# Plonky3/Plonky3-recursion

Hardware: AMD Instinct MI355X
Metric: prove_next_layer ms + Poseidon2 perms/s, KoalaBear 2^20-row circuit, 1/8 GPU (lower is better)
Workload: dtype u32 Montgomery (31-bit prime field, degree-4 extension); Poseidon2 hashing as exact integers in f64; 1 GPU; prove_next_layer (verifier-circuit run on the device + prove_all_tables) of the synthetic koala-bear 2^20-row recursion layer: tables const/public/alu/poseidon2/recompose, FRI blowup 4, arity<=4, 54 queries, 15-bit PoW; circuit inputs + NextLayerPrepCache resident in HBM; field=koala-bear, log_height=20, independent_proofs=1, proof_bytes=612900, parallelism=1 independent proofs, one per GPU, no data-path collective

## Files before the change

plonky3_recursion_amd/csrc/field.h:

```cpp
#pragma once
#include <type_traits>
#include <stdint.h>

#if defined(__HIPCC__)
#include <hip/hip_runtime.h>
#define P3R_HD __host__ __device__ __forceinline__
#else
#define P3R_HD inline
#endif

namespace p3r {

#if defined(__HIPCC__)
template <class T>
using gptr = T __attribute__((address_space(1)))*;
template <class T>
__device__ __forceinline__ gptr<T> as_global(T* p) {
  return (gptr<T>)p;
}

template <class Job>
__device__ __forceinline__ int find_job(const Job* __restrict__ jobs, int n_jobs) {
  int lo = 0, hi = n_jobs - 1;
  while (lo < hi) {
// ... 32 lines not shown
};
struct BabyBearParams {
  static constexpr uint32_t P = 0x78000001u;
  static constexpr uint32_t GEN = 31;
  static constexpr int TWO_ADICITY = 27;
  static constexpr uint32_t EXT_W = 11;
  static constexpr int SBOX_DEGREE = 7;
  static constexpr int SBOX_REGISTERS = 1;
  static constexpr int PARTIAL_ROUNDS = 13;
  static constexpr int PARTIAL_ROUNDS_W32 = 30;
  static constexpr int FIELD_ID = 1;
};

template <class PP>
struct Fp {
  using Params = PP;
  static constexpr uint32_t P = PP::P;
  static constexpr uint32_t MU = inv_mod_2_32(PP::P);
  static constexpr uint32_t R1 = (uint32_t)((1ull << 32) % PP::P);
  static constexpr uint32_t R2 = (uint32_t)((uint64_t)R1 * R1 % PP::P);

  uint32_t v;

  static P3R_HD uint32_t mulhi(uint32_t a, uint32_t b) {
#if defined(__HIP_DEVICE_COMPILE__)
    return __umulhi(a, b);
#else
    return (uint32_t)(((uint64_t)a * b) >> 32);
#endif
  }
  static constexpr uint32_t NEG_MU = 0u - MU;
  static P3R_HD uint32_t reduce64(uint64_t x) {
#if defined(__HIP_DEVICE_COMPILE__)
    const uint32_t q = (uint32_t)x * NEG_MU;
    const uint32_t r = (uint32_t)(((uint64_t)q * P + x) >> 32);
    const uint32_t r2 = r - P;
    return r < r2 ? r : r2;
#else
    const uint32_t lo = (uint32_t)x, hi = (uint32_t)(x >> 32);
    uint32_t t = lo * MU;
    uint32_t u = mulhi(t, P);
    uint32_t r = hi - u;
    return hi < u ? r + P : r;
#endif
  }
  static P3R_HD uint32_t reduce(uint32_t lo, uint32_t hi) { return reduce64(((uint64_t)hi << 32) | lo); }
  static P3R_HD uint32_t reduce64_lazy(uint64_t x) {
#if defined(__HIP_DEVICE_COMPILE__)
    const uint32_t q = (uint32_t)x * NEG_MU;
    return (uint32_t)(((uint64_t)q * P + x) >> 32);
#else
    return reduce64(x);
#endif
  }
  P3R_HD Fp sqr_times(Fp x) const {
    const uint32_t sq = reduce64_lazy((uint64_t)v * v);
    return raw(reduce64((uint64_t)sq * x.v));
  }
  P3R_HD Fp cube() const {
    const uint32_t sq = reduce64_lazy((uint64_t)v * v);
    return raw(reduce64((uint64_t)sq * v));
  }
  static P3R_HD Fp raw(uint32_t m) { Fp r; r.v = m; return r; }
  static P3R_HD Fp zero() { return raw(0); }
  static P3R_HD Fp one() { return raw(R1); }
  static P3R_HD Fp from_canonical(uint32_t x) {
    return raw(reduce64((uint64_t)x * R2));
  }
  static P3R_HD Fp from_u64(uint64_t x) { return from_canonical((uint32_t)(x % P)); }
  P3R_HD uint32_t to_canonical() const { return reduce(v, 0); }

  friend P3R_HD Fp operator+(Fp a, Fp b) {
    uint32_t s = a.v + b.v;
    return raw(s >= P ? s - P : s);
  }
  friend P3R_HD Fp operator-(Fp a, Fp b) {
    uint32_t d = a.v - b.v;
    return raw(a.v < b.v ? d + P : d);
  }
  friend P3R_HD Fp operator*(Fp a, Fp b) { return raw(reduce64((uint64_t)a.v * b.v)); }
  static P3R_HD Fp dot2(Fp a1, Fp b1, Fp a2, Fp b2) {
    return raw(reduce64((uint64_t)a1.v * b1.v + (uint64_t)a2.v * b2.v));
  }
  P3R_HD Fp operator-() const { return raw(v ? P - v : 0); }
  P3R_HD Fp& operator+=(Fp o) { *this = *this + o; return *this; }
  P3R_HD Fp& operator-=(Fp o) { *this = *this - o; return *this; }
  P3R_HD Fp& operator*=(Fp o) { *this = *this * o; return *this; }
  P3R_HD bool operator==(Fp o) const { return v == o.v; }
  P3R_HD bool operator!=(Fp o) const { return v != o.v; }
  P3R_HD Fp dbl() const { return *this + *this; }
  P3R_HD Fp sqr() const { return *this * *this; }
  P3R_HD Fp halve() const {
    uint32_t t = (v & 1) ? v + P : v;
    return raw(t >> 1);
  }
  P3R_HD Fp pow(uint64_t e) const {
    Fp r = one(), b = *this;
    while (e) {
      if (e & 1) r *= b;
      b = b.sqr();
      e >>= 1;
    }
    return r;
  }
  P3R_HD Fp inv() const { return pow((uint64_t)P - 2); }

  static P3R_HD Fp generator() { return from_canonical(PP::GEN); }
  static P3R_HD Fp two_adic_generator(int bits) {
    Fp g = from_canonical(PP::GEN).pow(((uint64_t)P - 1) >> PP::TWO_ADICITY);
    for (int i = PP::TWO_ADICITY; i > bits; --i) g = g.sqr();
    return g;
  }
};

template <class PP>
struct Fp4 {
  using F = Fp<PP>;
  F c[4];

  static P3R_HD Fp4 zero() { Fp4 r; r.c[0] = r.c[1] = r.c[2] = r.c[3] = F::zero(); return r; }
  static P3R_HD Fp4 one() { Fp4 r = zero(); r.c[0] = F::one(); return r; }
  static P3R_HD Fp4 from_base(F b) { Fp4 r = zero(); r.c[0] = b; return r; }
  static P3R_HD F w() { return F::from_canonical(PP::EXT_W); }

  friend P3R_HD Fp4 operator+(Fp4 a, Fp4 b) {
    Fp4 r;
    for (int i = 0; i < 4; ++i) r.c[i] = a.c[i] + b.c[i];
    return r;
  }
  friend P3R_HD Fp4 operator-(Fp4 a, Fp4 b) {
    Fp4 r;
    for (int i = 0; i < 4; ++i) r.c[i] = a.c[i] - b.c[i];
    return r;
  }
  P3R_HD Fp4 operator-() const {
    Fp4 r;
    for (int i = 0; i < 4; ++i) r.c[i] = -c[i];
    return r;
  }
  friend P3R_HD Fp4 operator*(Fp4 a, Fp4 b) {
    const F W = w();
    const F wa1 = W * a.c[1], wa2 = W * a.c[2], wa3 = W * a.c[3];
    Fp4 r;
    r.c[0] = F::dot2(a.c[0], b.c[0], wa1, b.c[3]) + F::dot2(wa2, b.c[2], wa3, b.c[1]);
    r.c[1] = F::dot2(a.c[0], b.c[1], a.c[1], b.c[0]) + F::dot2(wa2, b.c[3], wa3, b.c[2]);
    r.c[2] = F::dot2(a.c[0], b.c[2], a.c[1], b.c[1]) + F::dot2(a.c[2], b.c[0], wa3, b.c[3]);
    r.c[3] = F::dot2(a.c[0], b.c[3], a.c[1], b.c[2]) + F::dot2(a.c[2], b.c[1], a.c[3], b.c[0]);
    return r;
  }
  friend P3R_HD Fp4 operator*(Fp4 a, F b) {
    Fp4 r;
    for (int i = 0; i < 4; ++i) r.c[i] = a.c[i] * b;
    return r;
  }
  static P3R_HD Fp4 dot2_base(const Fp4& a1, F b1, const Fp4& a2, F b2) {
    Fp4 r;
    for (int i = 0; i < 4; ++i) r.c[i] = F::dot2(a1.c[i], b1, a2.c[i], b2);
    return r;
  }
  P3R_HD Fp4& operator+=(Fp4 o) { *this = *this + o; return *this; }
  P3R_HD Fp4& operator-=(Fp4 o) { *this = *this - o; return *this; }
  P3R_HD Fp4& operator*=(Fp4 o) { *this = *this * o; return *this; }
  P3R_HD bool operator==(const Fp4& o) const {
    return c[0] == o.c[0] && c[1] == o.c[1] && c[2] == o.c[2] && c[3] == o.c[3];
  }
  P3R_HD bool is_zero() const { return (c[0].v | c[1].v | c[2].v | c[3].v) == 0; }
  P3R_HD Fp4 sqr() const { return *this * *this; }
  P3R_HD Fp4 dbl() const { Fp4 r; for (int i = 0; i < 4; ++i) r.c[i] = c[i].dbl(); return r; }
  P3R_HD Fp4 halve() const { Fp4 r; for (int i = 0; i < 4; ++i) r.c[i] = c[i].halve(); return r; }
  P3R_HD Fp4 pow(uint64_t e) const {
    Fp4 r = one(), b = *this;
    while (e) {
      if (e & 1) r *= b;
      b = b.sqr();
      e >>= 1;
    }
    return r;
  }
  struct Norm { F n0, n1, d; };
  P3R_HD Norm norm() const {
    const F W = w();
    F A0 = c[0] * c[0] + W * (c[2] * c[2]);
    F A1 = (c[0] * c[2]).dbl();
    F B0 = c[1] * c[1] + W * (c[3] * c[3]);
    F B1 = (c[1] * c[3]).dbl();
    Norm r;
    r.n0 = A0 - W * B1;
    r.n1 = A1 - B0;
    r.d = r.n0 * r.n0 - W * (r.n1 * r.n1);
    return r;
  }
  P3R_HD Fp4 inv() const {
    const Norm nm = norm();
    return inv_given(nm, nm.d.inv());
  }
  P3R_HD Fp4 inv_given(const Norm& nm, F d) const {
    const F W = w();
    F i0 = nm.n0 * d;
    F i1 = -(nm.n1 * d);
    Fp4 r;
    r.c[0] = c[0] * i0 + W * (c[2] * i1);
    r.c[2] = c[0] * i1 + c[2] * i0;
    r.c[1] = -(c[1] * i0 + W * (c[3] * i1));
    r.c[3] = -(c[1] * i1 + c[3] * i0);
    return r;
  }
};

template <class PP>
inline constexpr bool kHasQuintic = PP::P == 0x7f000001u;
template <class PP>
struct Fp1 {
  using F = Fp<PP>;
  F c[1];
  static P3R_HD Fp1 zero() { Fp1 r; r.c[0] = F::zero(); return r; }
  friend P3R_HD Fp1 operator+(Fp1 a, Fp1 b) { Fp1 r; r.c[0] = a.c[0] + b.c[0]; return r; }
  friend P3R_HD Fp1 operator-(Fp1 a, Fp1 b) { Fp1 r; r.c[0] = a.c[0] - b.c[0]; return r; }
  friend P3R_HD Fp1 operator*(Fp1 a, Fp1 b) { Fp1 r; r.c[0] = a.c[0] * b.c[0]; return r; }
  static P3R_HD Fp1 one() { Fp1 r; r.c[0] = F::one(); return r; }
  static P3R_HD Fp1 from_base(F b) { Fp1 r; r.c[0] = b; return r; }
  P3R_HD bool operator==(const Fp1& o) const { return c[0] == o.c[0]; }
  P3R_HD Fp1 inv() const { Fp1 r; r.c[0] = c[0].inv(); return r; }
};
template <class PP, class Fn>
inline void dispatch_ext_degree(int d, Fn&& fn) {
  if (d == 1) fn(std::integral_constant<int, 1>{});
  else if (d == 5) { if constexpr (kHasQuintic<PP>) fn(std::integral_constant<int, 5>{}); }
  else fn(std::integral_constant<int, 4>{});
}
template <class PP, class Fn>
inline void dispatch_air_degree(int d, Fn&& fn) {
  if (d == 2) fn(std::integral_constant<int, 2>{});
  else if (d == 6) fn(std::integral_constant<int, 6>{});
  else if (d == 8) fn(std::integral_constant<int, 8>{});
  else dispatch_ext_degree<PP>(d, fn);
}
inline bool ext_degree_is_binomial_generic(uint32_t d) { return d == 2 || d == 6 || d == 8; }

namespace quintic {
struct Q5 { uint64_t c[5]; };
constexpr Q5 q5_mul(Q5 a, Q5 b, uint64_t p) {
  uint64_t t[9] = {0, 0, 0, 0, 0, 0, 0, 0, 0};
  for (int i = 0; i < 5; ++i)
    for (int j = 0; j < 5; ++j) t[i + j] = (t[i + j] + a.c[i] * b.c[j] % p) % p;
  for (int k = 8; k >= 5; --k) {
    t[k - 5] = (t[k - 5] + t[k]) % p;
    t[k - 3] = (t[k - 3] + p - t[k]) % p;
  }
  return Q5{{t[0], t[1], t[2], t[3], t[4]}};
}
constexpr Q5 q5_pow(Q5 b, uint64_t e, uint64_t p) {
  Q5 r{{1, 0, 0, 0, 0}};
  while (e) {
    if (e & 1) r = q5_mul(r, b, p);
    b = q5_mul(b, b, p);
    e >>= 1;
  }
  return r;
}
constexpr uint32_t frob_entry(uint32_t p, int k, int i, int j) {
  Q5 x{{0, 1, 0, 0, 0}};
  for (int s = 0; s < k; ++s) x = q5_pow(x, p, p);
  const Q5 xi = q5_pow(x, (uint64_t)i, p);
  return (uint32_t)((xi.c[j] << 32) % p);
}
}
template <class PP, int K, int I, int J>
inline constexpr uint32_t kFrob5 = quintic::frob_entry(PP::P, K, I, J);

template <class PP>
struct Fp5 {
  using F = Fp<PP>;
  F c[5];
  static P3R_HD Fp5 zero() { Fp5 r; for (int i = 0; i < 5; ++i) r.c[i] = F::zero(); return r; }
  friend P3R_HD Fp5 operator+(Fp5 a, Fp5 b) { Fp5 r; for (int i = 0; i < 5; ++i) r.c[i] = a.c[i] + b.c[i]; return r; }
  friend P3R_HD Fp5 operator-(Fp5 a, Fp5 b) { Fp5 r; for (int i = 0; i < 5; ++i) r.c[i] = a.c[i] - b.c[i]; return r; }
  friend P3R_HD Fp5 operator*(Fp5 a, Fp5 b) {
    const F c5 = F::dot2(a.c[1], b.c[4], a.c[2], b.c[3]) + F::dot2(a.c[3], b.c[2], a.c[4], b.c[1]);
    const F c6 = F::dot2(a.c[2], b.c[4], a.c[3], b.c[3]) + a.c[4] * b.c[2];
    const F c7 = F::dot2(a.c[3], b.c[4], a.c[4], b.c[3]);
    const F c8 = a.c[4] * b.c[4];
    const F c58 = c5 - c8;
    Fp5 r;
    r.c[0] = a.c[0] * b.c[0] + c58;
    r.c[1] = F::dot2(a.c[0], b.c[1], a.c[1], b.c[0]) + c6;
    r.c[2] = F::dot2(a.c[0], b.c[2], a.c[1], b.c[1]) + a.c[2] * b.c[0] - c58 + c7;
    r.c[3] = F::dot2(a.c[0], b.c[3], a.c[1], b.c[2]) + F::dot2(a.c[2], b.c[1], a.c[3], b.c[0]) - c6 + c8;
    r.c[4] = F::dot2(a.c[0], b.c[4], a.c[1], b.c[3]) + F::dot2(a.c[2], b.c[2], a.c[3], b.c[1]) + a.c[4] * b.c[0] - c7;
    return r;
  }
  friend P3R_HD Fp5 operator*(Fp5 a, F b) { Fp5 r; for (int i = 0; i < 5; ++i) r.c[i] = a.c[i] * b; return r; }
  P3R_HD Fp5 operator-() const { Fp5 r; for (int i = 0; i < 5; ++i) r.c[i] = -c[i]; return r; }
  P3R_HD Fp5& operator+=(Fp5 o) { *this = *this + o; return *this; }
  P3R_HD Fp5& operator-=(Fp5 o) { *this = *this - o; return *this; }
  P3R_HD Fp5& operator*=(Fp5 o) { *this = *this * o; return *this; }
  P3R_HD bool is_zero() const { return (c[0].v | c[1].v | c[2].v | c[3].v | c[4].v) == 0; }
  P3R_HD Fp5 sqr() const { return *this * *this; }
  P3R_HD Fp5 dbl() const { Fp5 r; for (int i = 0; i < 5; ++i) r.c[i] = c[i].dbl(); return r; }
  P3R_HD Fp5 halve() const { Fp5 r; for (int i = 0; i < 5; ++i) r.c[i] = c[i].halve(); return r; }
  P3R_HD Fp5 pow(uint64_t e) const {
    Fp5 r = one(), b = *this;
    while (e) {
      if (e & 1) r *= b;
      b = b.sqr();
      e >>= 1;
    }
    return r;
  }
  static P3R_HD Fp5 dot2_base(const Fp5& a1, F b1, const Fp5& a2, F b2) {
    Fp5 r;
    for (int i = 0; i < 5; ++i) r.c[i] = F::dot2(a1.c[i], b1, a2.c[i], b2);
    return r;
  }
  static P3R_HD Fp5 one() { Fp5 r = zero(); r.c[0] = F::one(); return r; }
  static P3R_HD Fp5 from_base(F b) { Fp5 r = zero(); r.c[0] = b; return r; }
  P3R_HD bool operator==(const Fp5& o) const {
    return c[0] == o.c[0] && c[1] == o.c[1] && c[2] == o.c[2] && c[3] == o.c[3] && c[4] == o.c[4];
  }
  template <int K, int J>
  P3R_HD F frobenius_coeff() const {
    const F t = F::dot2(c[1], F::raw(kFrob5<PP, K, 1, J>), c[2], F::raw(kFrob5<PP, K, 2, J>)) +
                F::dot2(c[3], F::raw(kFrob5<PP, K, 3, J>), c[4], F::raw(kFrob5<PP, K, 4, J>));
    return J == 0 ? c[0] + t : t;
  }
  template <int K>
  P3R_HD Fp5 frobenius() const {
    Fp5 r;
    r.c[0] = frobenius_coeff<K, 0>();
    r.c[1] = frobenius_coeff<K, 1>();
    r.c[2] = frobenius_coeff<K, 2>();
    r.c[3] = frobenius_coeff<K, 3>();
    r.c[4] = frobenius_coeff<K, 4>();
    return r;
  }
  static P3R_HD F mul_c0(const Fp5& a, const Fp5& b) {
    return a.c[0] * b.c[0] + F::dot2(a.c[1], b.c[4], a.c[2], b.c[3]) + F::dot2(a.c[3], b.c[2], a.c[4], b.c[1]) -
           a.c[4] * b.c[4];
  }
  P3R_HD Fp5 norm_cofactor() const {
    const Fp5 a1 = frobenius<1>();
    const Fp5 t = a1 * a1.template frobenius<1>();
    return t * t.template frobenius<2>();
  }
  P3R_HD Fp5 inv() const {
    const Fp5 co = norm_cofactor();
    return co * mul_c0(*this, co).inv();
  }
};

template <class PP, int D> struct CircuitExt;
template <class PP> struct CircuitExt<PP, 1> { using type = Fp1<PP>; };
template <class PP> struct CircuitExt<PP, 4> { using type = Fp4<PP>; };
template <class PP> struct CircuitExt<PP, 5> { using type = Fp5<PP>; };

template <class V> struct Lift;
template <class PP> struct Lift<Fp<PP>> { static P3R_HD Fp<PP> of(Fp<PP> x) { return x; } };
template <class PP> struct Lift<Fp4<PP>> { static P3R_HD Fp4<PP> of(Fp<PP> x) { return Fp4<PP>::from_base(x); } };
template <class PP> struct Lift<Fp5<PP>> { static P3R_HD Fp5<PP> of(Fp<PP> x) { return Fp5<PP>::from_base(x); } };
template <class PP, int DC> struct Chal;
template <class PP> struct Chal<PP, 4> { using type = Fp4<PP>; };
template <class PP> struct Chal<PP, 5> { using type = Fp5<PP>; };

P3R_HD uint32_t bit_reverse(uint32_t x, int bits) {
  if (bits == 0) return 0;
#if defined(__HIP_DEVICE_COMPILE__)
  return __brev(x) >> (32 - bits);
#else
  uint32_t r = 0;
  for (int i = 0; i < bits; ++i) r |= ((x >> i) & 1u) << (bits - 1 - i);
  return r;
#endif
}

}
```

plonky3_recursion_amd/csrc/field_test_ops.h:

```cpp
#pragma once
#include "field.h"

namespace p3r {

enum FieldTestOp : int {
  FT_FP_ADD = 0,
  FT_FP_SUB = 1,
  FT_FP_NEG = 2,
  FT_FP_MUL = 3,
  FT_FP_SQR = 4,
  FT_FP_DBL = 5,
  FT_FP_HALVE = 6,
  FT_FP_DOT2 = 7,
  FT_FP_SQR_TIMES = 8,
  FT_FP_CUBE = 9,
  FT_FP_REDUCE_LAZY = 10,
  FT_FP_FROM_CANONICAL = 11,
  FT_FP_TO_CANONICAL = 12,
  FT_FP_POW = 13,
  FT_FP_INV = 14,
  FT_FP_TWO_ADIC_GEN = 15,
  FT_BIT_REVERSE = 16,

  FT_FP4_ADD = 32,
  FT_FP4_SUB = 33,
  FT_FP4_NEG = 34,
  FT_FP4_MUL = 35,
  FT_FP4_MUL_BASE = 36,
  FT_FP4_DOT2_BASE = 37,
  FT_FP4_SQR = 38,
  FT_FP4_DBL = 39,
  FT_FP4_HALVE = 40,
  FT_FP4_POW = 41,
  FT_FP4_NORM = 42,
  FT_FP4_INV_GIVEN = 43,
  FT_FP4_INV = 44,

  FT_FP5_ADD = 64,
  FT_FP5_SUB = 65,
  FT_FP5_NEG = 66,
  FT_FP5_MUL = 67,
  FT_FP5_MUL_BASE = 68,
  FT_FP5_DOT2_BASE = 69,
  FT_FP5_SQR = 70,
  FT_FP5_FROBENIUS1 = 71,
  FT_FP5_FROBENIUS2 = 72,
  FT_FP5_MUL_C0 = 73,
  FT_FP5_NORM_COFACTOR = 74,
  FT_FP5_POW = 75,
  FT_FP5_INV = 76,
  FT_FP5_DBL = 77,
  FT_FP5_HALVE = 78,

  FT_FP1_MUL = 96,
  FT_FP1_INV = 97,
};

P3R_HD bool field_test_shape(int op, int* words_in, int* words_out) {
  int wi = 0, wo = 0;
  switch (op) {
    case FT_FP_ADD: case FT_FP_SUB: case FT_FP_MUL: case FT_FP_SQR_TIMES: case FT_FP_REDUCE_LAZY: case FT_BIT_REVERSE:
      wi = 2, wo = 1; break;
    case FT_FP_NEG: case FT_FP_SQR: case FT_FP_DBL: case FT_FP_HALVE: case FT_FP_CUBE: case FT_FP_FROM_CANONICAL:
    case FT_FP_TO_CANONICAL: case FT_FP_POW: case FT_FP_INV: case FT_FP_TWO_ADIC_GEN:
      wi = 1, wo = 1; break;
    case FT_FP_DOT2: wi = 4, wo = 1; break;
    case FT_FP4_ADD: case FT_FP4_SUB: case FT_FP4_MUL: wi = 8, wo = 4; break;
    case FT_FP4_NEG: case FT_FP4_SQR: case FT_FP4_DBL: case FT_FP4_HALVE: case FT_FP4_POW: case FT_FP4_INV: wi = 4, wo = 4; break;
    case FT_FP4_MUL_BASE: case FT_FP4_INV_GIVEN: wi = 5, wo = 4; break;
    case FT_FP4_DOT2_BASE: wi = 10, wo = 4; break;
    case FT_FP4_NORM: wi = 4, wo = 3; break;
    case FT_FP5_ADD: case FT_FP5_SUB: case FT_FP5_MUL: wi = 10, wo = 5; break;
    case FT_FP5_NEG: case FT_FP5_SQR: case FT_FP5_FROBENIUS1: case FT_FP5_FROBENIUS2: case FT_FP5_NORM_COFACTOR:
    case FT_FP5_POW: case FT_FP5_INV: case FT_FP5_DBL: case FT_FP5_HALVE:
      wi = 5, wo = 5; break;
    case FT_FP5_MUL_BASE: wi = 6, wo = 5; break;
    case FT_FP5_DOT2_BASE: wi = 12, wo = 5; break;
    case FT_FP5_MUL_C0: wi = 10, wo = 1; break;
    case FT_FP1_MUL: wi = 2, wo = 1; break;
    case FT_FP1_INV: wi = 1, wo = 1; break;
    default: return false;
  }
  *words_in = wi;
  *words_out = wo;
  return true;
}
P3R_HD bool field_test_is_quintic(int op) { return op >= FT_FP5_ADD && op <= FT_FP5_HALVE; }

template <class E, int D>
P3R_HD E field_test_load(const uint32_t* in) {
  E e;
  for (int i = 0; i < D; ++i) e.c[i].v = in[i];
  return e;
}
template <class E, int D>
P3R_HD void field_test_store(uint32_t* out, const E& e) {
  for (int i = 0; i < D; ++i) out[i] = e.c[i].v;
}

template <class PP>
P3R_HD bool field_test_apply(int op, const uint32_t* in, uint32_t* out, uint32_t aux) {
  using F = Fp<PP>;
  using E4 = Fp4<PP>;
  using E1 = Fp1<PP>;
  auto f = [&](int i) { return F::raw(in[i]); };
  auto e4 = [&](int i) { return field_test_load<E4, 4>(in + i); };
  auto put4 = [&](const E4& e) { field_test_store<E4, 4>(out, e); };
  switch (op) {
    case FT_FP_ADD: out[0] = (f(0) + f(1)).v; return true;
    case FT_FP_SUB: out[0] = (f(0) - f(1)).v; return true;
    case FT_FP_NEG: out[0] = (-f(0)).v; return true;
    case FT_FP_MUL: out[0] = (f(0) * f(1)).v; return true;
    case FT_FP_SQR: out[0] = f(0).sqr().v; return true;
    case FT_FP_DBL: out[0] = f(0).dbl().v; return true;
    case FT_FP_HALVE: out[0] = f(0).halve().v; return true;
    case FT_FP_DOT2: out[0] = F::dot2(f(0), f(1), f(2), f(3)).v; return true;
    case FT_FP_SQR_TIMES: out[0] = f(0).sqr_times(f(1)).v; return true;
    case FT_FP_CUBE: out[0] = f(0).cube().v; return true;
    case FT_FP_REDUCE_LAZY: out[0] = F::reduce64_lazy((uint64_t)in[0] * in[1]); return true;
    case FT_FP_FROM_CANONICAL: out[0] = F::from_canonical(in[0]).v; return true;
    case FT_FP_TO_CANONICAL: out[0] = f(0).to_canonical(); return true;
    case FT_FP_POW: out[0] = f(0).pow(aux).v; return true;
    case FT_FP_INV: out[0] = f(0).inv().v; return true;
    case FT_FP_TWO_ADIC_GEN: out[0] = F::two_adic_generator((int)in[0]).v; return true;
    case FT_BIT_REVERSE: out[0] = bit_reverse(in[0], (int)in[1]); return true;

    case FT_FP4_ADD: put4(e4(0) + e4(4)); return true;
    case FT_FP4_SUB: put4(e4(0) - e4(4)); return true;
    case FT_FP4_NEG: put4(-e4(0)); return true;
    case FT_FP4_MUL: put4(e4(0) * e4(4)); return true;
    case FT_FP4_MUL_BASE: put4(e4(0) * f(4)); return true;
    case FT_FP4_DOT2_BASE: put4(E4::dot2_base(e4(0), f(4), e4(5), f(9))); return true;
    case FT_FP4_SQR: put4(e4(0).sqr()); return true;
    case FT_FP4_DBL: put4(e4(0).dbl()); return true;
    case FT_FP4_HALVE: put4(e4(0).halve()); return true;
    case FT_FP4_POW: put4(e4(0).pow(aux)); return true;
    case FT_FP4_NORM: {
      const typename E4::Norm nm = e4(0).norm();
      out[0] = nm.n0.v, out[1] = nm.n1.v, out[2] = nm.d.v;
      return true;
    }
    case FT_FP4_INV_GIVEN: {
      const E4 a = e4(0);
      put4(a.inv_given(a.norm(), f(4)));
      return true;
    }
    case FT_FP4_INV: put4(e4(0).inv()); return true;

    case FT_FP1_MUL: field_test_store<E1, 1>(out, field_test_load<E1, 1>(in) * field_test_load<E1, 1>(in + 1)); return true;
    case FT_FP1_INV: field_test_store<E1, 1>(out, field_test_load<E1, 1>(in).inv()); return true;
    default: break;
  }
  if constexpr (kHasQuintic<PP>) {
    using E5 = Fp5<PP>;
    auto e5 = [&](int i) { return field_test_load<E5, 5>(in + i); };
    auto put5 = [&](const E5& e) { field_test_store<E5, 5>(out, e); };
    switch (op) {
      case FT_FP5_ADD: put5(e5(0) + e5(5)); return true;
      case FT_FP5_SUB: put5(e5(0) - e5(5)); return true;
      case FT_FP5_NEG: put5(-e5(0)); return true;
      case FT_FP5_MUL: put5(e5(0) * e5(5)); return true;
      case FT_FP5_MUL_BASE: put5(e5(0) * f(5)); return true;
      case FT_FP5_DOT2_BASE: put5(E5::dot2_base(e5(0), f(5), e5(6), f(11))); return true;
      case FT_FP5_SQR: put5(e5(0).sqr()); return true;
      case FT_FP5_FROBENIUS1: put5(e5(0).template frobenius<1>()); return true;
      case FT_FP5_FROBENIUS2: put5(e5(0).template frobenius<2>()); return true;
      case FT_FP5_MUL_C0: out[0] = E5::mul_c0(e5(0), e5(5)).v; return true;
      case FT_FP5_NORM_COFACTOR: put5(e5(0).norm_cofactor()); return true;
      case FT_FP5_POW: put5(e5(0).pow(aux)); return true;
      case FT_FP5_INV: put5(e5(0).inv()); return true;
      case FT_FP5_DBL: put5(e5(0).dbl()); return true;
      case FT_FP5_HALVE: put5(e5(0).halve()); return true;
      default: break;
    }
  }
  return false;
}

}
```

plonky3_recursion_amd/csrc/kernels_fri_points.hip.h:

```cpp
#pragma once
#include "kernels_fri_reduce.hip.h"

namespace p3r {

template <int DC>
struct FriPointT {
  const uint32_t* inv;
  const uint32_t* v;
  EW<DC> off;
};
struct FriPointsMat {
  const uint32_t* mat;
  int w;
  uint32_t p0, n_points;
};
template <class PP, int DC = 4>
__global__ void __launch_bounds__(kBlock)
k_fri_reduce_points(const FriReduceJob* __restrict__ jobs, int n_jobs, const FriPointsMat* __restrict__ mats,
                    const FriPointT<DC>* __restrict__ pts, const uint32_t* __restrict__ apow_tab ) {
  using F = Fp<PP>;
  using E = typename Chal<PP, DC>::type;
  const int j = find_job(jobs, n_jobs);
  const FriReduceJob job = jobs[j];
  const size_t h = job.h, r = (size_t)(blockIdx.x - job.block0) * kBlock + threadIdx.x;
  if (r >= h) return;
  auto apow = [&](int c) {
    E ap;
#pragma unroll
    for (int k = 0; k < DC; ++k) ap.c[k] = F::raw(apow_tab[DC * c + k]);
    return ap;
  };
  E acc = E::zero();
  for (uint32_t m = 0; m < job.n_mats; ++m) {
    const FriPointsMat a = mats[job.mat0 + m];
    const gptr<const uint32_t> mat = as_global(a.mat);
    const int w = a.w;
    E S = E::zero(), S2 = E::zero();
    int c = 0;
    for (; c + 3 < w; c += 4) {
      const F m0 = F::raw(mat[(size_t)c * h + r]), m1 = F::raw(mat[(size_t)(c + 1) * h + r]);
      const F m2 = F::raw(mat[(size_t)(c + 2) * h + r]), m3 = F::raw(mat[(size_t)(c + 3) * h + r]);
      S += E::dot2_base(apow(c), m0, apow(c + 1), m1);
      S2 += E::dot2_base(apow(c + 2), m2, apow(c + 3), m3);
    }
    for (; c + 1 < w; c += 2)
      S += E::dot2_base(apow(c), F::raw(mat[(size_t)c * h + r]), apow(c + 1), F::raw(mat[(size_t)(c + 1) * h + r]));
    if (c < w) S += apow(c) * F::raw(mat[(size_t)c * h + r]);
    S += S2;
    for (uint32_t p = 0; p < a.n_points; ++p) {
      const FriPointT<DC>& q = pts[a.p0 + p];
      E inv, V;
#pragma unroll
      for (int k = 0; k < DC; ++k) inv.c[k] = F::raw(as_global(q.inv)[(size_t)k * h + r]);
#pragma unroll
      for (int k = 0; k < DC; ++k) V.c[k] = F::raw(as_global(q.v)[k]);
      acc += e4_load<PP, DC>(q.off) * (V - S) * inv;
    }
  }
#pragma unroll
  for (int k = 0; k < DC; ++k) as_global(job.ro)[(size_t)k * h + r] = acc.c[k].v;
}

template <int DC, int LA>
__global__ void __launch_bounds__(kBlock) k_fri_leaf_view(const uint32_t* __restrict__ in, uint32_t* __restrict__ out, size_t rows) {
  static_assert(LA >= 1 && LA <= 4, "rows of 2, 4, 8 or 16 elements");
  constexpr int ARITY = 1 << LA;
  const size_t r = (size_t)blockIdx.x * kBlock + threadIdx.x;
  const int k = (int)blockIdx.y;
  if (r >= rows) return;
  const size_t n_in = rows << LA;
  const gptr<const uint32_t> src = as_global(in) + (size_t)k * n_in + (r << LA);
  uint32_t e[ARITY];
  if constexpr (LA == 1) {
    const fri_u32x2 v = *(gptr<const fri_u32x2>)src;
    e[0] = v.x;
    e[1] = v.y;
  } else {
#pragma unroll
    for (int q = 0; q < ARITY / 4; ++q) {
      const fri_u32x4 v = ((gptr<const fri_u32x4>)src)[q];
      e[4 * q] = v.x;
      e[4 * q + 1] = v.y;
      e[4 * q + 2] = v.z;
      e[4 * q + 3] = v.w;
    }
  }
  const gptr<uint32_t> dst = as_global(out) + (size_t)k * rows + r;
#pragma unroll
  for (int j = 0; j < ARITY; ++j) dst[(size_t)j * DC * rows] = e[j];
}

}
```

plonky3_recursion_amd/csrc/kernels_fri_reduce.hip.h:

```cpp
#pragma once
#include "kernels_stark.hip.h"

namespace p3r {

template <int DC>
struct FriInvJobT {
  uint32_t* inv;
  uint64_t h;
  int log_h;
  uint32_t w_h;
  uint32_t w_4;
  EW<DC> z;
  uint32_t block0;
};
using FriInvJob = FriInvJobT<4>;
template <class PP, int DC = 4>
__global__ void __launch_bounds__(kBlock)
k_fri_inv_points(const FriInvJobT<DC>* __restrict__ jobs, int n_jobs, uint32_t gen) {
  using F = Fp<PP>;
  using E = typename Chal<PP, DC>::type;
  const int j = find_job(jobs, n_jobs);
  const FriInvJobT<DC>& job = jobs[j];
  const size_t h = job.h, r0 = ((size_t)(blockIdx.x - job.block0) * kBlock + threadIdx.x) * 4;
  if (r0 >= h) return;
  const E z = e4_load<PP, DC>(job.z);
  E x[4], v[4];
  const F x0 = F::raw(gen) * F::raw(job.w_h).pow(bit_reverse((uint32_t)r0, job.log_h));
  const F x2 = x0 * F::raw(job.w_4);
  x[0] = z - E::from_base(x0);
  x[1] = z + E::from_base(x0);
  x[2] = z - E::from_base(x2);
  x[3] = z + E::from_base(x2);
  inv4<PP>(x, v);
  const gptr<uint32_t> inv = as_global(job.inv);
#pragma unroll
  for (int m = 0; m < 4; ++m)
    if (r0 + m < h)
#pragma unroll
      for (int k = 0; k < DC; ++k) inv[(size_t)k * h + r0 + m] = v[m].c[k].v;
}

struct FriVsumJob {
  const uint32_t* vals;
  uint32_t* out;
  int w;
};
template <class PP, int DC = 4>
__global__ void __launch_bounds__(kBlock)
k_fri_vsum(const FriVsumJob* __restrict__ jobs, const uint32_t* __restrict__ apow_tab ) {
  using F = Fp<PP>;
  using E = typename Chal<PP, DC>::type;
  __shared__ uint32_t sh[kBlock / 64][DC];
  const FriVsumJob job = jobs[blockIdx.x];
  const gptr<const uint32_t> vals = as_global(job.vals);
  E acc = E::zero();
  for (int c = threadIdx.x; c < job.w; c += kBlock) {
    E ap, v;
#pragma unroll
    for (int k = 0; k < DC; ++k) {
      ap.c[k] = F::raw(apow_tab[DC * c + k]);
      v.c[k] = F::raw(vals[DC * c + k]);
    }
    acc += ap * v;
  }
  const int lane = threadIdx.x & 63, wave = threadIdx.x >> 6;
#pragma unroll
  for (int k = 0; k < DC; ++k) {
    F x = acc.c[k];
#pragma unroll
    for (int off = 32; off > 0; off >>= 1) x += F::raw(__shfl_down(x.v, off));
    if (lane == 0) sh[wave][k] = x.v;
  }
  __syncthreads();
  if (threadIdx.x < DC) {
    F x = F::zero();
#pragma unroll
    for (int wv = 0; wv < kBlock / 64; ++wv) x += F::raw(sh[wv][threadIdx.x]);
    as_global(job.out)[threadIdx.x] = x.v;
  }
}

template <int DC>
struct FriReduceMatT {
  const uint32_t* mat;
  int w, n_points;
  const uint32_t* inv[2];
  const uint32_t* v[2];
  EW<DC> off[2];
};
using FriReduceMat = FriReduceMatT<4>;
struct FriReduceJob {
  uint32_t* ro;
  uint64_t h;
  uint32_t mat0, n_mats;
  uint32_t block0;
};
template <class PP, int DC = 4>
__global__ void __launch_bounds__(kBlock)
k_fri_reduce_pre(const FriReduceJob* __restrict__ jobs, int n_jobs, const FriReduceMatT<DC>* __restrict__ mats,
                 const uint32_t* __restrict__ apow_tab ) {
  using F = Fp<PP>;
  using E = typename Chal<PP, DC>::type;
  const int j = find_job(jobs, n_jobs);
  const FriReduceJob job = jobs[j];
  const size_t h = job.h, r = (size_t)(blockIdx.x - job.block0) * kBlock + threadIdx.x;
  if (r >= h) return;
  auto apow = [&](int c) {
    E ap;
#pragma unroll
    for (int k = 0; k < DC; ++k) ap.c[k] = F::raw(apow_tab[DC * c + k]);
    return ap;
  };
  E acc = E::zero();
  for (uint32_t m = 0; m < job.n_mats; ++m) {
    const FriReduceMatT<DC>& a = mats[job.mat0 + m];
    const gptr<const uint32_t> mat = as_global(a.mat);
    const int w = a.w;
    E S = E::zero(), S2 = E::zero();
    int c = 0;
    for (; c + 3 < w; c += 4) {
      const F m0 = F::raw(mat[(size_t)c * h + r]), m1 = F::raw(mat[(size_t)(c + 1) * h + r]);
      const F m2 = F::raw(mat[(size_t)(c + 2) * h + r]), m3 = F::raw(mat[(size_t)(c + 3) * h + r]);
      S += E::dot2_base(apow(c), m0, apow(c + 1), m1);
      S2 += E::dot2_base(apow(c + 2), m2, apow(c + 3), m3);
    }
    for (; c + 1 < w; c += 2)
      S += E::dot2_base(apow(c), F::raw(mat[(size_t)c * h + r]), apow(c + 1), F::raw(mat[(size_t)(c + 1) * h + r]));
    if (c < w) S += apow(c) * F::raw(mat[(size_t)c * h + r]);
    S += S2;
    for (int p = 0; p < a.n_points; ++p) {
      E inv;
#pragma unroll
      for (int k = 0; k < DC; ++k) inv.c[k] = F::raw(as_global(a.inv[p])[(size_t)k * h + r]);
      E V;
#pragma unroll
      for (int k = 0; k < DC; ++k) V.c[k] = F::raw(as_global(a.v[p])[k]);
      acc += e4_load<PP, DC>(a.off[p]) * (V - S) * inv;
    }
  }
#pragma unroll
  for (int k = 0; k < DC; ++k) as_global(job.ro)[(size_t)k * h + r] = acc.c[k].v;
}

}
```

plonky3_recursion_amd/csrc/prove_impl.hip.h:

```cpp
#include "host_transcript.h"
#include "kernels_stark.hip.h"
#include "kernels_fri_reduce.hip.h"
#include "kernels_zk.hip.h"
#include "open_impl.hip.h"

struct p3r_prep {
  std::vector<p3r::AirParams> airs;
  std::vector<std::unique_ptr<p3r_dmat>> traces;
  std::vector<std::unique_ptr<p3r_dmat>> evals;
  std::vector<std::unique_ptr<p3r_dmat>> ldes;
  std::vector<size_t> heights;
  int zk_codewords = -1;
  const p3r_dmat* committed(size_t i) const { return evals.empty() ? traces[i].get() : evals[i].get(); }
  std::unique_ptr<p3r_tree> tree;
  std::vector<uint32_t> cap_canonical;
};

namespace {

template <class PP, int DC = 4>
EW<DC> to_e4(const typename Chal<PP, DC>::type& e) { return e4_store<PP, DC>(e); }

template <class PP, int DC = 4>
std::vector<typename Chal<PP, DC>::type> download_ef(p3r_ctx* ctx, const uint32_t* dev, size_t count) {
// ... 640 lines not shown
    P3R_HIP(ctx->stage.upload(ctx->stream, inv_keep.back().p, inv_jobs.data(), inv_jobs.size() * sizeof(FriInvJobT<DC>)));
    ProfScope ps(ctx, "fri_inv_points");
    hipLaunchKernelGGL((k_fri_inv_points<PP, DC>), dim3(inv_blocks), dim3(kBlock), 0, ctx->stream,
                       reinterpret_cast<const FriInvJobT<DC>*>(inv_keep.back().p), (int)inv_jobs.size(), gen.v);
    P3R_HIP(hipGetLastError());
  }

  void check_at_zeta() {
    E l_beta_pow[kMaxExtD + 1];
    for (int j = 0; j <= kMaxExtD; ++j) l_beta_pow[j] = e4_load<PP, DC>(lc.beta_pow[j]);
    const E l_prefix = e4_load<PP, DC>(lc.prefix);
    std::vector<std::vector<std::vector<E>>> inst_chunks(ni);
    for (const Mat& m : quot_round.mats) inst_chunks[m.inst].push_back(m.vals[0]);
    static const std::vector<E> empty;
    for (size_t i = 0; i < ni; ++i) {
      const auto& omain = main_round.mats[i].vals;
      const Mat* pm = perm_mat(i);
      ZetaInstance<PP, DC> zi{&omain[0], omain.size() > 1 ? &omain[1] : nullptr, &prep_round.mats[i].vals[0],
                          &prep_round.mats[i].vals[1], pm ? &pm->vals[0] : &empty, pm ? &pm->vals[1] : &empty,
                          &inst_chunks[i], pm ? &terminals[i] : nullptr};
      try {
        check_instance_at_zeta<PP, DC>(prep->airs[i], layouts[i], log_n[i], zi, alpha, zeta, l_prefix, l_beta_pow,
                                   ctx->rc_mont_host.data(), i, zk);
      } catch (const VerifyFailure& e) {
        fail(P3R_EINVAL, "the traces do not satisfy the constraints (%s)", e.what());
      }
    }
    E tsum = E::zero();
    for (const Mat& m : perm_round.mats) tsum += terminals[m.inst];
    if (!tsum.is_zero()) fail(P3R_EINVAL, "the traces do not satisfy the constraints (global lookup sum is not zero)");
  }

  void fri_reduce() {
    prof_stage(ctx, "fri_reduce");
    const E fri_alpha = ch.sample_ext();
    size_t max_w = 1, n_opened = 0;
    for (Round* r : rounds())
      for (const Mat& m : r->mats) { max_w = std::max(max_w, m.lde->w); ++n_opened; }
    std::vector<E> fa_pow(max_w + 1);
    fa_pow[0] = E::one();
    for (size_t c = 1; c <= max_w; ++c) fa_pow[c] = fa_pow[c - 1] * fri_alpha;
    d_fapow.alloc(max_w * DC);
    {
      std::vector<uint32_t> h(max_w * DC);
      for (size_t c = 0; c < max_w; ++c)
        for (int k = 0; k < DC; ++k) h[c * DC + k] = fa_pow[c].c[k].v;
      P3R_HIP(ctx->stage.upload(ctx->stream, d_fapow.p, h.data(), h.size() * 4));
    }
    std::map<int, std::vector<FriReduceMatT<DC>>> by_height;
    std::vector<DevBuf> keep;
    std::vector<FriVsumJob> vsum_jobs;
    DevBuf vsums(2 * DC * n_opened);
    for (Round* r : rounds())
      for (const Mat& m : r->mats) {
        const int lh = log_e[m.inst] + log_blowup;
        auto f = ros.find(lh);
        if (f == ros.end()) f = ros.emplace(lh, std::make_pair(E::one(), DevBuf((size_t)DC << lh))).first;
        FriReduceMatT<DC> a{};
        a.mat = m.lde->d;
        a.w = (int)m.lde->w;
        a.n_points = (int)m.z.size();
        E ap = f->second.first;
        for (size_t p = 0; p < m.z.size(); ++p) {
          a.inv[p] = inv_cache.at(inv_key(lh, m.z[p]));
          a.v[p] = vsums.p + DC * vsum_jobs.size();
          vsum_jobs.push_back({op.values_dev(m.job, (int)p), vsums.p + DC * vsum_jobs.size(), (int)m.ev->w});
          a.off[p] = to_e4<PP, DC>(ap);
          ap *= fa_pow[m.lde->w];
        }
        f->second.first = ap;
        by_height[lh].push_back(a);
      }
    std::vector<FriReduceMatT<DC>> mats;
    std::vector<FriReduceJob> jobs;
    uint32_t blocks = 0;
    for (auto& kv : by_height) {
      FriReduceJob j{};
      j.ro = ros[kv.first].second.p;
      j.h = uint64_t(1) << kv.first;
      j.mat0 = (uint32_t)mats.size();
      j.n_mats = (uint32_t)kv.second.size();
      j.block0 = blocks;
      blocks += blocks_for(size_t(1) << kv.first);
      jobs.push_back(j);
      mats.insert(mats.end(), kv.second.begin(), kv.second.end());
    }
    const size_t b_mats = mats.size() * sizeof(FriReduceMatT<DC>), b_jobs = jobs.size() * sizeof(FriReduceJob),
                 b_vsum = vsum_jobs.size() * sizeof(FriVsumJob);
    const size_t o_jobs = (b_mats + 15) & ~size_t(15), o_vsum = (o_jobs + b_jobs + 15) & ~size_t(15);
    std::vector<unsigned char> blob(o_vsum + b_vsum);
    std::memcpy(blob.data(), mats.data(), b_mats);
    std::memcpy(blob.data() + o_jobs, jobs.data(), b_jobs);
    std::memcpy(blob.data() + o_vsum, vsum_jobs.data(), b_vsum);
    keep.emplace_back((blob.size() + 3) / 4);
    unsigned char* d_blob = reinterpret_cast<unsigned char*>(keep.back().p);
    P3R_HIP(ctx->stage.upload(ctx->stream, d_blob, blob.data(), blob.size()));
    const auto* d_mats = reinterpret_cast<const FriReduceMatT<DC>*>(d_blob);
    const auto* d_jobs = reinterpret_cast<const FriReduceJob*>(d_blob + o_jobs);
    const auto* d_vsum = reinterpret_cast<const FriVsumJob*>(d_blob + o_vsum);
    {
      ProfScope ps(ctx, "fri_reduce");
      hipLaunchKernelGGL((k_fri_vsum<PP, DC>), dim3((unsigned)vsum_jobs.size()), dim3(kBlock), 0, ctx->stream, d_vsum,
                         d_fapow.p);
      hipLaunchKernelGGL((k_fri_reduce_pre<PP, DC>), dim3(blocks), dim3(kBlock), 0, ctx->stream, d_jobs, (int)jobs.size(),
                         d_mats, d_fapow.p);
    }
    P3R_HIP(hipGetLastError());
  }

  void fri_commit_phase() {
    prof_stage(ctx, "fri_commit_phase");
    std::vector<int> heights;
    for (auto& kv : ros) heights.push_back(kv.first);
    std::sort(heights.rbegin(), heights.rend());
    log_max = heights[0];
    const int log_final = (int)cfg.log_final_poly_len + log_blowup;
    folded = std::move(ros[log_max].second);
    size_t next_h = 1;
    int log_cur = log_max;
    const bool device_transcript = cfg.cap_height == 0 && cfg.commit_pow_bits == 0 && ch.in_buf.empty();
    d_tstate.alloc(P2_WIDTH);
    d_phase.alloc((DC + P2_DIGEST) * kMaxPhases);
    uint32_t* const d_betas = d_phase.p;
    uint32_t* const d_caps = d_phase.p + DC * kMaxPhases;
    if (device_transcript) {
      uint32_t st[P2_WIDTH];
      for (int k = 0; k < P2_WIDTH; ++k) st[k] = ch.state[k].v;
      P3R_HIP(ctx->stage.upload(ctx->stream, d_tstate.p, st, sizeof st));
    }
    while (log_cur > log_final) {
      int log_next = next_h < heights.size() ? heights[next_h] : -1;
      int la = fri_log_arity(ctx->fri_log_arities, phases.size(), (int)cfg.max_log_arity, log_cur, log_final, log_next);
      if (la < 0) fail(P3R_EINVAL, "fri_log_arities does not fit the proof: phase %zu at height 2^%d", phases.size(), log_cur);
      if (la > 4) fail(P3R_EUNSUPPORTED, "max_log_arity > 4 is not supported");
      const size_t arity = size_t(1) << la, rows = (size_t(1) << log_cur) >> la;
      Phase ph{la, rows};
      commit_phase_leaves(ph, log_cur);
      const size_t pi = phases.size();
      if (pi >= kMaxPhases) fail(P3R_EUNSUPPORTED, "more than %zu FRI commit phases", kMaxPhases);
      TranscriptStep step{d_tstate.p, d_betas + DC * pi, d_caps + P2_DIGEST * pi};
      step.dc = DC;
      mmcs_build_levels<PP>(ctx, ph.tree.get(), nullptr, device_transcript ? &step : nullptr);
      if (device_transcript) {
        if (!step.done)
          hipLaunchKernelGGL(k_fri_transcript_step<PP>, dim3(1), dim3(64), 0, ctx->stream, ph.tree->layers.back().p,
                             step.state, step.beta, step.cap, ctx->rc.p, ctx->p2_diag.p, DC);
      } else {
        ph.cap = mmcs_cap_mont(ctx, ph.tree.get());
        for (uint32_t v : ph.cap) ch.observe(F::raw(v));
        commit_pow_witnesses.push_back(grind_witness<PP>(ctx, ch, (int)cfg.commit_pow_bits));
        const E beta = ch.sample_ext();
        uint32_t bw[DC];
        for (int k = 0; k < DC; ++k) bw[k] = beta.c[k].v;
        P3R_HIP(ctx->stage.upload(ctx->stream, d_betas + DC * pi, bw, sizeof bw));
      }
      DevBuf out(DC * rows);
      FriFoldArgs fa{};
      fa.in = folded.p; fa.out = out.p; fa.rows = rows; fa.log_rows = log_cur - la;
      fa.beta = d_betas + DC * pi;
      const bool roll = next_h < heights.size() && heights[next_h] == log_cur - la;
      fa.roll = roll ? ros[heights[next_h]].second.p : nullptr;
      fa.w_inv = F::two_adic_generator(log_cur).inv().v;
      const F omega = F::two_adic_generator(la);
      for (int s = 0; s < la; ++s) {
        F om_s = omega.pow(uint64_t(1) << s);
        for (int j = 0; j < (int)(arity >> (s + 1)); ++j)
// ... 301 lines not shown
```

Measured before the change: 25.97 ms.

## Use dot4 lazy reduction and hoist per-point inverse multiply out of FRI reduce

Adds a four-term base-field dot product that reduces once per four products, and uses it in the FRI reduce and FRI points column loops. In k_fri_reduce_pre, when all matrices of a height share at most two distinct inverse-denominator arrays, the terms are accumulated per point and multiplied by the inverse once at the end. This removes repeated loads of the inverse columns and repeated extension multiplies per matrix. It also adds a launch-bounds occupancy hint of 8 and a host-side slot assignment, at the cost of extra accumulator registers.

After: 25.97 ms. About the same (+0.0%).

```diff
diff --git a/plonky3_recursion_amd/csrc/field.h b/plonky3_recursion_amd/csrc/field.h
--- a/plonky3_recursion_amd/csrc/field.h
+++ b/plonky3_recursion_amd/csrc/field.h
@@ -138,6 +138,13 @@
   static P3R_HD Fp dot2(Fp a1, Fp b1, Fp a2, Fp b2) {
     return raw(reduce64((uint64_t)a1.v * b1.v + (uint64_t)a2.v * b2.v));
   }
+  static_assert((uint64_t)(PP::P - 1) * (PP::P - 1) < (uint64_t(1) << 62), "dot4: 4*(P-1)^2 < 2^64, the sum fits a u64");
+  static_assert((uint64_t)PP::P * PP::P <= ((uint64_t)PP::P << 31), "dot4: 4*P^2 <= 2P*2^32, one subtraction of P*2^32 suffices");
+  static P3R_HD Fp dot4(Fp a1, Fp b1, Fp a2, Fp b2, Fp a3, Fp b3, Fp a4, Fp b4) {
+    const uint64_t s = (uint64_t)a1.v * b1.v + (uint64_t)a2.v * b2.v + (uint64_t)a3.v * b3.v + (uint64_t)a4.v * b4.v;
+    const uint32_t hi = (uint32_t)(s >> 32), hi2 = hi - P;
+    return raw(reduce(uint32_t(s), hi < hi2 ? hi : hi2));
+  }
   P3R_HD Fp operator-() const { return raw(v ? P - v : 0); }
   P3R_HD Fp& operator+=(Fp o) { *this = *this + o; return *this; }
   P3R_HD Fp& operator-=(Fp o) { *this = *this - o; return *this; }
@@ -212,6 +219,11 @@
   static P3R_HD Fp4 dot2_base(const Fp4& a1, F b1, const Fp4& a2, F b2) {
     Fp4 r;
     for (int i = 0; i < 4; ++i) r.c[i] = F::dot2(a1.c[i], b1, a2.c[i], b2);
+    return r;
+  }
+  static P3R_HD Fp4 dot4_base(const Fp4& a1, F b1, const Fp4& a2, F b2, const Fp4& a3, F b3, const Fp4& a4, F b4) {
+    Fp4 r;
+    for (int i = 0; i < 4; ++i) r.c[i] = F::dot4(a1.c[i], b1, a2.c[i], b2, a3.c[i], b3, a4.c[i], b4);
     return r;
   }
   P3R_HD Fp4& operator+=(Fp4 o) { *this = *this + o; return *this; }
@@ -368,6 +380,11 @@
     for (int i = 0; i < 5; ++i) r.c[i] = F::dot2(a1.c[i], b1, a2.c[i], b2);
     return r;
   }
+  static P3R_HD Fp5 dot4_base(const Fp5& a1, F b1, const Fp5& a2, F b2, const Fp5& a3, F b3, const Fp5& a4, F b4) {
+    Fp5 r;
+    for (int i = 0; i < 5; ++i) r.c[i] = F::dot4(a1.c[i], b1, a2.c[i], b2, a3.c[i], b3, a4.c[i], b4);
+    return r;
+  }
   static P3R_HD Fp5 one() { Fp5 r = zero(); r.c[0] = F::one(); return r; }
   static P3R_HD Fp5 from_base(F b) { Fp5 r = zero(); r.c[0] = b; return r; }
   P3R_HD bool operator==(const Fp5& o) const {
diff --git a/plonky3_recursion_amd/csrc/field_test_ops.h b/plonky3_recursion_amd/csrc/field_test_ops.h
--- a/plonky3_recursion_amd/csrc/field_test_ops.h
+++ b/plonky3_recursion_amd/csrc/field_test_ops.h
@@ -21,6 +21,7 @@
   FT_FP_INV = 14,
   FT_FP_TWO_ADIC_GEN = 15,
   FT_BIT_REVERSE = 16,
+  FT_FP_DOT4 = 17,
 
   FT_FP4_ADD = 32,
   FT_FP4_SUB = 33,
@@ -35,6 +36,7 @@
   FT_FP4_NORM = 42,
   FT_FP4_INV_GIVEN = 43,
   FT_FP4_INV = 44,
+  FT_FP4_DOT4_BASE = 45,
 
   FT_FP5_ADD = 64,
   FT_FP5_SUB = 65,
@@ -51,6 +53,7 @@
   FT_FP5_INV = 76,
   FT_FP5_DBL = 77,
   FT_FP5_HALVE = 78,
+  FT_FP5_DOT4_BASE = 79,
 
   FT_FP1_MUL = 96,
   FT_FP1_INV = 97,
@@ -65,10 +68,12 @@
     case FT_FP_TO_CANONICAL: case FT_FP_POW: case FT_FP_INV: case FT_FP_TWO_ADIC_GEN:
       wi = 1, wo = 1; break;
     case FT_FP_DOT2: wi = 4, wo = 1; break;
+    case FT_FP_DOT4: wi = 8, wo = 1; break;
     case FT_FP4_ADD: case FT_FP4_SUB: case FT_FP4_MUL: wi = 8, wo = 4; break;
     case FT_FP4_NEG: case FT_FP4_SQR: case FT_FP4_DBL: case FT_FP4_HALVE: case FT_FP4_POW: case FT_FP4_INV: wi = 4, wo = 4; break;
     case FT_FP4_MUL_BASE: case FT_FP4_INV_GIVEN: wi = 5, wo = 4; break;
     case FT_FP4_DOT2_BASE: wi = 10, wo = 4; break;
+    case FT_FP4_DOT4_BASE: wi = 20, wo = 4; break;
     case FT_FP4_NORM: wi = 4, wo = 3; break;
     case FT_FP5_ADD: case FT_FP5_SUB: case FT_FP5_MUL: wi = 10, wo = 5; break;
     case FT_FP5_NEG: case FT_FP5_SQR: case FT_FP5_FROBENIUS1: case FT_FP5_FROBENIUS2: case FT_FP5_NORM_COFACTOR:
@@ -76,6 +81,7 @@
       wi = 5, wo = 5; break;
     case FT_FP5_MUL_BASE: wi = 6, wo = 5; break;
     case FT_FP5_DOT2_BASE: wi = 12, wo = 5; break;
+    case FT_FP5_DOT4_BASE: wi = 24, wo = 5; break;
     case FT_FP5_MUL_C0: wi = 10, wo = 1; break;
     case FT_FP1_MUL: wi = 2, wo = 1; break;
     case FT_FP1_INV: wi = 1, wo = 1; break;
@@ -85,7 +91,7 @@
   *words_out = wo;
   return true;
 }
-P3R_HD bool field_test_is_quintic(int op) { return op >= FT_FP5_ADD && op <= FT_FP5_HALVE; }
+P3R_HD bool field_test_is_quintic(int op) { return op >= FT_FP5_ADD && op <= FT_FP5_DOT4_BASE; }
 
 template <class E, int D>
 P3R_HD E field_test_load(const uint32_t* in) {
@@ -115,6 +121,7 @@
     case FT_FP_DBL: out[0] = f(0).dbl().v; return true;
     case FT_FP_HALVE: out[0] = f(0).halve().v; return true;
     case FT_FP_DOT2: out[0] = F::dot2(f(0), f(1), f(2), f(3)).v; return true;
+    case FT_FP_DOT4: out[0] = F::dot4(f(0), f(1), f(2), f(3), f(4), f(5), f(6), f(7)).v; return true;
     case FT_FP_SQR_TIMES: out[0] = f(0).sqr_times(f(1)).v; return true;
     case FT_FP_CUBE: out[0] = f(0).cube().v; return true;
     case FT_FP_REDUCE_LAZY: out[0] = F::reduce64_lazy((uint64_t)in[0] * in[1]); return true;
@@ -131,6 +138,7 @@
     case FT_FP4_MUL: put4(e4(0) * e4(4)); return true;
     case FT_FP4_MUL_BASE: put4(e4(0) * f(4)); return true;
     case FT_FP4_DOT2_BASE: put4(E4::dot2_base(e4(0), f(4), e4(5), f(9))); return true;
+    case FT_FP4_DOT4_BASE: put4(E4::dot4_base(e4(0), f(4), e4(5), f(9), e4(10), f(14), e4(15), f(19))); return true;
     case FT_FP4_SQR: put4(e4(0).sqr()); return true;
     case FT_FP4_DBL: put4(e4(0).dbl()); return true;
     case FT_FP4_HALVE: put4(e4(0).halve()); return true;
@@ -162,6 +170,7 @@
       case FT_FP5_MUL: put5(e5(0) * e5(5)); return true;
       case FT_FP5_MUL_BASE: put5(e5(0) * f(5)); return true;
       case FT_FP5_DOT2_BASE: put5(E5::dot2_base(e5(0), f(5), e5(6), f(11))); return true;
+      case FT_FP5_DOT4_BASE: put5(E5::dot4_base(e5(0), f(5), e5(6), f(11), e5(12), f(17), e5(18), f(23))); return true;
       case FT_FP5_SQR: put5(e5(0).sqr()); return true;
       case FT_FP5_FROBENIUS1: put5(e5(0).template frobenius<1>()); return true;
       case FT_FP5_FROBENIUS2: put5(e5(0).template frobenius<2>()); return true;
diff --git a/plonky3_recursion_amd/csrc/kernels_fri_points.hip.h b/plonky3_recursion_amd/csrc/kernels_fri_points.hip.h
--- a/plonky3_recursion_amd/csrc/kernels_fri_points.hip.h
+++ b/plonky3_recursion_amd/csrc/kernels_fri_points.hip.h
@@ -37,14 +37,23 @@
     const int w = a.w;
     E S = E::zero(), S2 = E::zero();
     int c = 0;
-    for (; c + 3 < w; c += 4) {
-      const F m0 = F::raw(mat[(size_t)c * h + r]), m1 = F::raw(mat[(size_t)(c + 1) * h + r]);
-      const F m2 = F::raw(mat[(size_t)(c + 2) * h + r]), m3 = F::raw(mat[(size_t)(c + 3) * h + r]);
-      S += E::dot2_base(apow(c), m0, apow(c + 1), m1);
-      S2 += E::dot2_base(apow(c + 2), m2, apow(c + 3), m3);
+    auto four = [&](int c0) {
+      const F m0 = F::raw(mat[(size_t)c0 * h + r]), m1 = F::raw(mat[(size_t)(c0 + 1) * h + r]);
+      const F m2 = F::raw(mat[(size_t)(c0 + 2) * h + r]), m3 = F::raw(mat[(size_t)(c0 + 3) * h + r]);
+      return E::dot4_base(apow(c0), m0, apow(c0 + 1), m1, apow(c0 + 2), m2, apow(c0 + 3), m3);
+    };
+    for (; c + 7 < w; c += 8) {
+      S += four(c);
+      S2 += four(c + 4);
     }
-    for (; c + 1 < w; c += 2)
-      S += E::dot2_base(apow(c), F::raw(mat[(size_t)c * h + r]), apow(c + 1), F::raw(mat[(size_t)(c + 1) * h + r]));
+    if (c + 3 < w) {
+      S += four(c);
+      c += 4;
+    }
+    if (c + 1 < w) {
+      S2 += E::dot2_base(apow(c), F::raw(mat[(size_t)c * h + r]), apow(c + 1), F::raw(mat[(size_t)(c + 1) * h + r]));
+      c += 2;
+    }
     if (c < w) S += apow(c) * F::raw(mat[(size_t)c * h + r]);
     S += S2;
     for (uint32_t p = 0; p < a.n_points; ++p) {
diff --git a/plonky3_recursion_amd/csrc/kernels_fri_reduce.hip.h b/plonky3_recursion_amd/csrc/kernels_fri_reduce.hip.h
--- a/plonky3_recursion_amd/csrc/kernels_fri_reduce.hip.h
+++ b/plonky3_recursion_amd/csrc/kernels_fri_reduce.hip.h
@@ -87,6 +87,7 @@
   const uint32_t* inv[2];
   const uint32_t* v[2];
   EW<DC> off[2];
+  int slot[2];
 };
 using FriReduceMat = FriReduceMatT<4>;
 struct FriReduceJob {
@@ -94,9 +95,11 @@
   uint64_t h;
   uint32_t mat0, n_mats;
   uint32_t block0;
+  uint32_t n_inv;
+  const uint32_t* inv[2];
 };
 template <class PP, int DC = 4>
-__global__ void __launch_bounds__(kBlock)
+__global__ void __launch_bounds__(kBlock, 8)
 k_fri_reduce_pre(const FriReduceJob* __restrict__ jobs, int n_jobs, const FriReduceMatT<DC>* __restrict__ mats,
                  const uint32_t* __restrict__ apow_tab ) {
   using F = Fp<PP>;
@@ -111,32 +114,52 @@
     for (int k = 0; k < DC; ++k) ap.c[k] = F::raw(apow_tab[DC * c + k]);
     return ap;
   };
-  E acc = E::zero();
+  auto load_inv = [&](const uint32_t* v) {
+    E inv;
+#pragma unroll
+    for (int k = 0; k < DC; ++k) inv.c[k] = F::raw(as_global(v)[(size_t)k * h + r]);
+    return inv;
+  };
+  const bool per_point = job.n_inv != 0;
+  E acc = E::zero(), pacc0 = E::zero(), pacc1 = E::zero();
   for (uint32_t m = 0; m < job.n_mats; ++m) {
     const FriReduceMatT<DC>& a = mats[job.mat0 + m];
     const gptr<const uint32_t> mat = as_global(a.mat);
     const int w = a.w;
     E S = E::zero(), S2 = E::zero();
     int c = 0;
-    for (; c + 3 < w; c += 4) {
-      const F m0 = F::raw(mat[(size_t)c * h + r]), m1 = F::raw(mat[(size_t)(c + 1) * h + r]);
-      const F m2 = F::raw(mat[(size_t)(c + 2) * h + r]), m3 = F::raw(mat[(size_t)(c + 3) * h + r]);
-      S += E::dot2_base(apow(c), m0, apow(c + 1), m1);
-      S2 += E::dot2_base(apow(c + 2), m2, apow(c + 3), m3);
+    auto four = [&](int c0) {
+      const F m0 = F::raw(mat[(size_t)c0 * h + r]), m1 = F::raw(mat[(size_t)(c0 + 1) * h + r]);
+      const F m2 = F::raw(mat[(size_t)(c0 + 2) * h + r]), m3 = F::raw(mat[(size_t)(c0 + 3) * h + r]);
+      return E::dot4_base(apow(c0), m0, apow(c0 + 1), m1, apow(c0 + 2), m2, apow(c0 + 3), m3);
+    };
+    for (; c + 7 < w; c += 8) {
+      S += four(c);
+      S2 += four(c + 4);
     }
-    for (; c + 1 < w; c += 2)
-      S += E::dot2_base(apow(c), F::raw(mat[(size_t)c * h + r]), apow(c + 1), F::raw(mat[(size_t)(c + 1) * h + r]));
+    if (c + 3 < w) {
+      S += four(c);
+      c += 4;
+    }
+    if (c + 1 < w) {
+      S2 += E::dot2_base(apow(c), F::raw(mat[(size_t)c * h + r]), apow(c + 1), F::raw(mat[(size_t)(c + 1) * h + r]));
+      c += 2;
+    }
     if (c < w) S += apow(c) * F::raw(mat[(size_t)c * h + r]);
     S += S2;
     for (int p = 0; p < a.n_points; ++p) {
-      E inv;
-#pragma unroll
-      for (int k = 0; k < DC; ++k) inv.c[k] = F::raw(as_global(a.inv[p])[(size_t)k * h + r]);
       E V;
 #pragma unroll
       for (int k = 0; k < DC; ++k) V.c[k] = F::raw(as_global(a.v[p])[k]);
-      acc += e4_load<PP, DC>(a.off[p]) * (V - S) * inv;
+      const E t = e4_load<PP, DC>(a.off[p]) * (V - S);
+      if (!per_point) acc += t * load_inv(a.inv[p]);
+      else if (a.slot[p] == 0) pacc0 += t;
+      else pacc1 += t;
     }
+  }
+  if (per_point) {
+    acc = pacc0 * load_inv(job.inv[0]);
+    if (job.n_inv > 1) acc += pacc1 * load_inv(job.inv[1]);
   }
 #pragma unroll
   for (int k = 0; k < DC; ++k) as_global(job.ro)[(size_t)k * h + r] = acc.c[k].v;
diff --git a/plonky3_recursion_amd/csrc/prove_impl.hip.h b/plonky3_recursion_amd/csrc/prove_impl.hip.h
--- a/plonky3_recursion_amd/csrc/prove_impl.hip.h
+++ b/plonky3_recursion_amd/csrc/prove_impl.hip.h
@@ -746,6 +746,17 @@
       j.n_mats = (uint32_t)kv.second.size();
       j.block0 = blocks;
       blocks += blocks_for(size_t(1) << kv.first);
+      std::vector<const uint32_t*> distinct;
+      for (FriReduceMatT<DC>& a : kv.second)
+        for (int p = 0; p < a.n_points; ++p) {
+          const size_t s = std::find(distinct.begin(), distinct.end(), a.inv[p]) - distinct.begin();
+          if (s == distinct.size()) distinct.push_back(a.inv[p]);
+          a.slot[p] = (int)s;
+        }
+      if (!distinct.empty() && distinct.size() <= 2) {
+        j.n_inv = (uint32_t)distinct.size();
+        for (size_t s = 0; s < distinct.size(); ++s) j.inv[s] = distinct[s];
+      }
       jobs.push_back(j);
       mats.insert(mats.end(), kv.second.begin(), kv.second.end());
     }
```
